# MasterBin-IIAU/Unicorn

Measured on NVIDIA H100. Metric: frames/sec, higher is better.
Workload: dtype bf16

## Files before the change

unicorn_b200/csrc/mlp_fused.cu:

```cuda
#include <algorithm>
#include "uc_ptx.cuh"
#include "uc_common.h"
#include "../../include/unicorn_b200.h"
#include "uc_epilogue.cuh"

namespace uc {

constexpr int kMlpRows = 128;
constexpr int kMlpHC = 64;
constexpr int kMlpConsumers = 2;
constexpr int kMlpThreads = (1 + kMlpConsumers) * 128;

template <int C>
struct MlpCfg {
  static constexpr int KB = (C + 63) / 64;
  static constexpr int A_BYTES = KB * kMlpRows * 128;
  static constexpr int W1_BYTES = KB * kMlpHC * 128;
  static constexpr int NH = C > 256 ? 2 : 1;
  static constexpr int N2 = C / NH;
  static constexpr int W2_BYTES = N2 * 128;
  static constexpr int NCHUNK = 4 * C / kMlpHC;
  static constexpr int STEPS = NH * NCHUNK;
  static constexpr int AS = C <= 192 ? 2 : 1;
  static constexpr int WS = C <= 256 ? 2 : 1;
  static constexpr int SMEM = AS * A_BYTES + WS * (W1_BYTES + W2_BYTES) + 1024 + 512;
  static constexpr int CPT = C / 16;
};

struct alignas(64) MlpParams {
  CUtensorMap tmA, tmW1, tmW2;
  const float* c1;
  const float* b2;
  const float* gamma;
  uint16_t* x;
  int M, m_tiles;
  float ln_eps;
};

enum { A_FULL = 0, A_EMPTY = 2, W1_FULL = 4, W1_EMPTY = 6, W2_FULL = 8, W2_EMPTY = 10, MLP_NBARS = 12 };

template <int C>
__global__ void __launch_bounds__(kMlpThreads, 1) convnext_mlp_kernel(const __grid_constant__ MlpParams p) {
  using Cfg = MlpCfg<C>;
  extern __shared__ uint8_t smem_raw[];
  uint8_t* smem = reinterpret_cast<uint8_t*>((reinterpret_cast<uintptr_t>(smem_raw) + 1023) & ~uintptr_t(1023));
  uint8_t* sA = smem;
  uint8_t* sW1 = sA + Cfg::AS * Cfg::A_BYTES;
  uint8_t* sW2 = sW1 + Cfg::WS * Cfg::W1_BYTES;
  uint64_t* bar = reinterpret_cast<uint64_t*>(sW2 + Cfg::WS * Cfg::W2_BYTES);
  const int wg = threadIdx.x >> 7, warp = threadIdx.x >> 5, lane = threadIdx.x & 31;

  if (threadIdx.x == 0) {
    prefetch_tmap(&p.tmA);
    prefetch_tmap(&p.tmW1);
    prefetch_tmap(&p.tmW2);
    for (int i = 0; i < 2; ++i) {
      mbar_init(&bar[A_FULL + i], 1);
      mbar_init(&bar[A_EMPTY + i], kMlpConsumers);
      mbar_init(&bar[W1_FULL + i], 1);
      mbar_init(&bar[W1_EMPTY + i], kMlpConsumers);
      mbar_init(&bar[W2_FULL + i], 1);
      mbar_init(&bar[W2_EMPTY + i], kMlpConsumers);
    }
    fence_barrier_init();
  }
  __syncthreads();
  pdl_wait();
  pdl_launch_dependents();

  const int n_local = (p.m_tiles - static_cast<int>(blockIdx.x) + static_cast<int>(gridDim.x) - 1) / static_cast<int>(gridDim.x);
  auto tile_of = [&](int i) { return static_cast<int>(blockIdx.x) + i * static_cast<int>(gridDim.x); };

  if (wg == 0) {
    regs_dealloc<40>();
    if (warp != 0) return;
    auto load_a = [&](int i) {
      const int ab = i % Cfg::AS;
      mbar_wait(&bar[A_EMPTY + ab], ((i / Cfg::AS) & 1) ^ 1);
      if (elect_one()) {
        mbar_arrive_expect_tx(&bar[A_FULL + ab], Cfg::A_BYTES);
#pragma unroll
        for (int kb = 0; kb < Cfg::KB; ++kb)
          tma_load_2d(sA + ab * Cfg::A_BYTES + kb * (kMlpRows * 128), &p.tmA, &bar[A_FULL + ab], kb * 64, tile_of(i) * kMlpRows);
      }
      __syncwarp();
    };
    auto load_w = [&](int g) {
      const int s = g % Cfg::WS, ph = (g / Cfg::WS) & 1, j = g % Cfg::NCHUNK, nh = (g / Cfg::NCHUNK) % Cfg::NH;
      mbar_wait(&bar[W1_EMPTY + s], ph ^ 1);
      if (elect_one()) {
        mbar_arrive_expect_tx(&bar[W1_FULL + s], Cfg::W1_BYTES);
#pragma unroll
        for (int kb = 0; kb < Cfg::KB; ++kb)
          tma_load_2d(sW1 + s * Cfg::W1_BYTES + kb * (kMlpHC * 128), &p.tmW1, &bar[W1_FULL + s], kb * 64, j * kMlpHC);
      }
      __syncwarp();
      mbar_wait(&bar[W2_EMPTY + s], ph ^ 1);
      if (elect_one()) {
        mbar_arrive_expect_tx(&bar[W2_FULL + s], Cfg::W2_BYTES);
        tma_load_2d(sW2 + s * Cfg::W2_BYTES, &p.tmW2, &bar[W2_FULL + s], j * kMlpHC, nh * Cfg::N2);
      }
      __syncwarp();
    };
    const int total = n_local * Cfg::STEPS;
    if (n_local > 0) load_a(0);
    for (int g = 0; g < total; ++g) {
      load_w(g);
      const int i = g / Cfg::STEPS, r = g % Cfg::STEPS;
      if (r == (Cfg::AS == 2 ? 0 : Cfg::STEPS - 1) && i + 1 < n_local) load_a(i + 1);
    }
    return;
  }
  regs_alloc<232>();
  const int c = wg - 1, ct = threadIdx.x & 127;
  const int g8 = lane >> 2, t = lane & 3;
  const int rl = (warp & 3) * 16 + g8;
  const int lr = c * 64 + (ct >> 1), lp = ct & 1;
  auto layer_norm_tile = [&](int ab) {
    uint8_t* a = sA + ab * Cfg::A_BYTES + lr * 128;
    auto chunk_ptr = [&](int cc) {
      const int gc = lp * Cfg::CPT + cc;
      return reinterpret_cast<uint4*>(a + (gc >> 3) * (kMlpRows * 128) + (((gc & 7) ^ (lr & 7)) << 4));
    };
    float s1 = 0.f;
#pragma unroll 4
    for (int cc = 0; cc < Cfg::CPT; ++cc) {
      const uint4 v = *chunk_ptr(cc);
      s1 += (bf16lo(v.x) + bf16hi(v.x)) + (bf16lo(v.y) + bf16hi(v.y)) + (bf16lo(v.z) + bf16hi(v.z)) + (bf16lo(v.w) + bf16hi(v.w));
    }
    s1 += __shfl_xor_sync(0xffffffffu, s1, 1);
    const float mean = s1 * (1.f / C);
    float s2 = 0.f;
#pragma unroll 4
    for (int cc = 0; cc < Cfg::CPT; ++cc) {
      const uint4 v = *chunk_ptr(cc);
      const uint32_t w[4] = {v.x, v.y, v.z, v.w};
#pragma unroll
      for (int e = 0; e < 4; ++e) {
        const float d0 = bf16lo(w[e]) - mean, d1 = bf16hi(w[e]) - mean;
        s2 = fmaf(d0, d0, s2);
        s2 = fmaf(d1, d1, s2);
      }
    }
    s2 += __shfl_xor_sync(0xffffffffu, s2, 1);
    const float rstd = rsqrtf(s2 * (1.f / C) + p.ln_eps);
#pragma unroll 4
    for (int cc = 0; cc < Cfg::CPT; ++cc) {
      uint4* ptr = chunk_ptr(cc);
      const uint4 v = *ptr;
      const uint32_t w[4] = {v.x, v.y, v.z, v.w};
      uint32_t o[4];
#pragma unroll
      for (int e = 0; e < 4; ++e) o[e] = pack2_fast((bf16lo(w[e]) - mean) * rstd, (bf16hi(w[e]) - mean) * rstd, false);
      *ptr = make_uint4(o[0], o[1], o[2], o[3]);
    }
    fence_proxy_async();
    named_sync(1 + c, 128);
  };
  const uint64_t a_desc0 = wgmma_desc_sw128(smem_u32(sA + c * 64 * 128)), w1_desc0 = wgmma_desc_sw128(smem_u32(sW1));
  const uint64_t w2_desc0 = wgmma_desc_sw128(smem_u32(sW2));
  float acc2[Cfg::N2 / 2];
  int g = 0;
  for (int i = 0; i < n_local; ++i) {
    const int ab = i % Cfg::AS;
    mbar_wait(&bar[A_FULL + ab], (i / Cfg::AS) & 1);
    layer_norm_tile(ab);
#pragma unroll 1
   for (int nh = 0; nh < Cfg::NH; ++nh) {
    for (int j = 0; j < Cfg::NCHUNK; ++j, ++g) {
      const int ws = g % Cfg::WS, wph = (g / Cfg::WS) & 1;
      float acc1[kMlpHC / 2];
      mbar_wait(&bar[W1_FULL + ws], wph);
      wgmma_fence();
#pragma unroll
      for (int kb = 0; kb < Cfg::KB; ++kb) {
        const uint64_t ad = a_desc0 + static_cast<uint64_t>((ab * Cfg::A_BYTES + kb * (kMlpRows * 128)) >> 4);
        const uint64_t bd = w1_desc0 + static_cast<uint64_t>((ws * Cfg::W1_BYTES + kb * (kMlpHC * 128)) >> 4);
#pragma unroll
        for (int k = 0; k < 4; ++k) wgmma_ss<kMlpHC, false>(acc1, ad + 2 * k, bd + 2 * k, (kb | k) != 0 ? 1u : 0u);
      }
      wgmma_commit();
      wgmma_wait<0>();
      wgmma_fence_regs(acc1);
      if (ct == 0) {
        mbar_arrive(&bar[W1_EMPTY + ws]);
        if (nh == Cfg::NH - 1 && j == Cfg::NCHUNK - 1) mbar_arrive(&bar[A_EMPTY + ab]);
      }
      uint32_t hf[4][4];
#pragma unroll
      for (int kk = 0; kk < 4; ++kk) {
#pragma unroll
        for (int half = 0; half < 2; ++half) {
          const int i8 = 2 * kk + half;
          const float2 bb = __ldg(reinterpret_cast<const float2*>(p.c1 + j * kMlpHC + 8 * i8 + 2 * t));
          const f32x2 h0 = gelu2(add2(pk2(acc1[4 * i8], acc1[4 * i8 + 1]), pk2(bb.x, bb.y)));
          const f32x2 h1 = gelu2(add2(pk2(acc1[4 * i8 + 2], acc1[4 * i8 + 3]), pk2(bb.x, bb.y)));
          hf[kk][2 * half] = pack2_fast(lo2(h0), hi2(h0), false);
          hf[kk][2 * half + 1] = pack2_fast(lo2(h1), hi2(h1), false);
        }
      }
      mbar_wait(&bar[W2_FULL + ws], wph);
      wgmma_fence();
      const uint64_t bd2 = w2_desc0 + static_cast<uint64_t>((ws * Cfg::W2_BYTES) >> 4);
#pragma unroll
      for (int kk = 0; kk < 4; ++kk) wgmma_rs_bf16<Cfg::N2>(acc2, hf[kk], bd2 + 2 * kk, (j | kk) != 0 ? 1u : 0u);
      wgmma_commit();
      wgmma_wait<0>();
      wgmma_fence_regs(acc2);
      if (ct == 0) mbar_arrive(&bar[W2_EMPTY + ws]);
    }
    const long grow0 = static_cast<long>(tile_of(i)) * kMlpRows + c * 64 + rl;
#pragma unroll
    for (int i8 = 0; i8 < Cfg::N2 / 8; ++i8) {
      const int col = nh * Cfg::N2 + 8 * i8 + 2 * t;
      const float2 b = __ldg(reinterpret_cast<const float2*>(p.b2 + col)), gm = __ldg(reinterpret_cast<const float2*>(p.gamma + col));
#pragma unroll
      for (int h = 0; h < 2; ++h) {
        const long grow = grow0 + 8 * h;
        if (grow < p.M) {
          uint32_t* xp = reinterpret_cast<uint32_t*>(p.x + grow * C + col);
          const uint32_t rw = *xp;
          f32x2 v = add2(pk2(acc2[4 * i8 + 2 * h], acc2[4 * i8 + 2 * h + 1]), pk2(b.x, b.y));
          v = mul2(v, pk2(gm.x, gm.y));
          v = add2(v, pk2(bf16lo(rw), bf16hi(rw)));
          *xp = pack2_fast(lo2(v), hi2(v), false);
        }
      }
    }
   }
  }
}

template <int C>
static int launch_mlp(MlpParams& p, cudaStream_t stream) {
  using Cfg = MlpCfg<C>;
  static PerDeviceFlag attr_dev;
  bool& attr = attr_dev.get();
  auto kern = convnext_mlp_kernel<C>;
  if (!attr) {
    cudaError_t e = cudaFuncSetAttribute(kern, cudaFuncAttributeMaxDynamicSharedMemorySize, Cfg::SMEM);
    if (e != cudaSuccess) return set_error(static_cast<int>(e), "uc_convnext_mlp: cudaFuncSetAttribute: %s", cudaGetErrorString(e));
    attr = true;
  }
  const int grid = std::min(p.m_tiles, num_sms());
  cudaError_t e = launch_pdl(kern, dim3(grid), dim3(kMlpThreads), Cfg::SMEM, stream, p);
  if (e != cudaSuccess) return set_error(static_cast<int>(e), "uc_convnext_mlp<%d> launch: %s", C, cudaGetErrorString(e));
  return check_launch("uc_convnext_mlp");
}

}

using namespace uc;

extern "C" int uc_convnext_mlp_supported(int C) { return C == 96 || C == 192 || C == 256 || C == 384; }

extern "C" int uc_convnext_mlp(const void* t_bf16, const void* w1f_bf16, const float* c1, const void* w2_bf16, const float* b2,
                               const float* gamma, void* x_bf16, int M, int C, float ln_eps, void* stream_v) {
  cudaStream_t stream = static_cast<cudaStream_t>(stream_v);
  if (!t_bf16 || !w1f_bf16 || !c1 || !w2_bf16 || !b2 || !gamma || !x_bf16) return set_error(UC_EINVAL, "uc_convnext_mlp: null pointer");
  if (!uc_convnext_mlp_supported(C)) return set_error(UC_EINVAL, "uc_convnext_mlp: C = %d not supported (96, 192, 256, 384)", C);
  if (M < 1) return set_error(UC_EINVAL, "uc_convnext_mlp: empty map");
  if ((reinterpret_cast<uintptr_t>(t_bf16) | reinterpret_cast<uintptr_t>(w1f_bf16) | reinterpret_cast<uintptr_t>(w2_bf16)) & 15 ||
      (reinterpret_cast<uintptr_t>(x_bf16) | reinterpret_cast<uintptr_t>(c1) | reinterpret_cast<uintptr_t>(b2) | reinterpret_cast<uintptr_t>(gamma)) & 31)
    return set_error(UC_EINVAL, "uc_convnext_mlp: t / weights 16-byte, x / biases 32-byte aligned");
  if (t_bf16 == x_bf16) return set_error(UC_EINVAL, "uc_convnext_mlp: t and x must be different maps");
  int rc = ensure_driver();
  if (rc) return rc;
  MlpParams p;
  memset(&p, 0, sizeof(p));
  const uint64_t es = 2;
  {
    uint64_t dims[2] = {static_cast<uint64_t>(C), static_cast<uint64_t>(M)};
    uint64_t strides[1] = {static_cast<uint64_t>(C) * es};
    uint32_t box[2] = {64, kMlpRows};
    rc = encode_tmap(&p.tmA, CU_TENSOR_MAP_DATA_TYPE_BFLOAT16, 2, t_bf16, dims, strides, box);
    if (rc) return rc;
  }
  {
    uint64_t dims[2] = {static_cast<uint64_t>(C), static_cast<uint64_t>(4 * C)};
    uint64_t strides[1] = {static_cast<uint64_t>(C) * es};
    uint32_t box[2] = {64, kMlpHC};
    rc = encode_tmap(&p.tmW1, CU_TENSOR_MAP_DATA_TYPE_BFLOAT16, 2, w1f_bf16, dims, strides, box);
    if (rc) return rc;
  }
  {
    uint64_t dims[2] = {static_cast<uint64_t>(4 * C), static_cast<uint64_t>(C)};
    uint64_t strides[1] = {static_cast<uint64_t>(4 * C) * es};
    uint32_t box[2] = {kMlpHC, static_cast<uint32_t>(C > 256 ? C / 2 : C)};
    rc = encode_tmap(&p.tmW2, CU_TENSOR_MAP_DATA_TYPE_BFLOAT16, 2, w2_bf16, dims, strides, box);
    if (rc) return rc;
  }
  p.c1 = c1; p.b2 = b2; p.gamma = gamma;
  p.x = static_cast<uint16_t*>(x_bf16);
  p.M = M;
  p.m_tiles = (M + kMlpRows - 1) / kMlpRows;
  p.ln_eps = ln_eps;
  return C == 96 ? launch_mlp<96>(p, stream) : C == 192 ? launch_mlp<192>(p, stream) : C == 256 ? launch_mlp<256>(p, stream) : launch_mlp<384>(p, stream);
}
```

unicorn_b200/csrc/uc_ptx.cuh:

```cuda
#pragma once
#include <cuda_runtime.h>
#include <cuda_bf16.h>
#include <cuda_fp16.h>
#include <cuda.h>
#include <stdint.h>
#include <stdio.h>
#include "uc_wgmma.cuh"

namespace uc {

__device__ __forceinline__ uint32_t smem_u32(const void* p) {
  return static_cast<uint32_t>(__cvta_generic_to_shared(p));
}

__device__ __forceinline__ bool elect_one() {
  uint32_t pred;
  asm volatile(
      "{\n\t.reg .pred p;\n\t"
      "elect.sync _|p, 0xffffffff;\n\t"
      "selp.u32 %0, 1, 0, p;\n\t}"
      : "=r"(pred));
  return pred != 0;
}

__device__ __forceinline__ void mbar_init(uint64_t* bar, uint32_t count) {
  asm volatile("mbarrier.init.shared::cta.b64 [%0], %1;" ::"r"(smem_u32(bar)), "r"(count) : "memory");
}
__device__ __forceinline__ void fence_barrier_init() {
  asm volatile("fence.mbarrier_init.release.cluster;" ::: "memory");
}
__device__ __forceinline__ void fence_proxy_async() {
  asm volatile("fence.proxy.async.shared::cta;" ::: "memory");
}
__device__ __forceinline__ void mbar_arrive_expect_tx(uint64_t* bar, uint32_t bytes) {
  asm volatile("mbarrier.arrive.expect_tx.shared::cta.b64 _, [%0], %1;" ::"r"(smem_u32(bar)), "r"(bytes)
               : "memory");
}
__device__ __forceinline__ void mbar_arrive(uint64_t* bar) {
  asm volatile("mbarrier.arrive.shared::cta.b64 _, [%0];" ::"r"(smem_u32(bar)) : "memory");
}
__device__ __forceinline__ bool mbar_try_wait(uint64_t* bar, uint32_t parity) {
  uint32_t ok;
  asm volatile(
      "{\n\t.reg .pred p;\n\t"
      "mbarrier.try_wait.parity.shared::cta.b64 p, [%1], %2;\n\t"
      "selp.u32 %0, 1, 0, p;\n\t}"
      : "=r"(ok)
      : "r"(smem_u32(bar)), "r"(parity)
      : "memory");
  return ok != 0;
}
__device__ __forceinline__ void mbar_wait(uint64_t* bar, uint32_t parity) {
  if (mbar_try_wait(bar, parity)) return;
  long long t0 = clock64();
  uint32_t spins = 0;
  while (!mbar_try_wait(bar, parity)) {
    if ((++spins & 0x3FF) == 0 && (clock64() - t0) > 4000000000LL) __trap();
  }
}

__device__ __forceinline__ void prefetch_tmap(const CUtensorMap* m) {
  asm volatile("prefetch.tensormap [%0];" ::"l"(reinterpret_cast<uint64_t>(m)) : "memory");
}
__device__ __forceinline__ void tma_load_2d(void* smem, const CUtensorMap* m, uint64_t* bar, int c0, int c1) {
  asm volatile(
      "cp.async.bulk.tensor.2d.shared::cluster.global.mbarrier::complete_tx::bytes [%0], [%1, {%3, %4}], [%2];" ::"r"(
          smem_u32(smem)),
      "l"(reinterpret_cast<uint64_t>(m)), "r"(smem_u32(bar)), "r"(c0), "r"(c1)
      : "memory");
}
__device__ __forceinline__ void tma_load_3d(void* smem, const CUtensorMap* m, uint64_t* bar, int c0, int c1, int c2) {
  asm volatile(
      "cp.async.bulk.tensor.3d.shared::cluster.global.mbarrier::complete_tx::bytes [%0], [%1, {%3, %4, %5}], [%2];" ::
          "r"(smem_u32(smem)),
      "l"(reinterpret_cast<uint64_t>(m)), "r"(smem_u32(bar)), "r"(c0), "r"(c1), "r"(c2)
      : "memory");
}
__device__ __forceinline__ void tma_load_4d(void* smem, const CUtensorMap* m, uint64_t* bar, int c0, int c1, int c2,
                                            int c3) {
  asm volatile(
      "cp.async.bulk.tensor.4d.shared::cluster.global.mbarrier::complete_tx::bytes [%0], [%1, {%3, %4, %5, %6}], "
      "[%2];" ::"r"(smem_u32(smem)),
      "l"(reinterpret_cast<uint64_t>(m)), "r"(smem_u32(bar)), "r"(c0), "r"(c1), "r"(c2), "r"(c3)
      : "memory");
}

__device__ __forceinline__ void tma_load_3d_mc(void* smem, const CUtensorMap* m, uint64_t* bar, int c0, int c1, int c2,
                                               uint16_t cta_mask) {
  asm volatile(
      "cp.async.bulk.tensor.3d.shared::cluster.global.mbarrier::complete_tx::bytes.multicast::cluster [%0], [%1, {%3, %4, "
      "%5}], [%2], %6;" ::"r"(smem_u32(smem)),
      "l"(reinterpret_cast<uint64_t>(m)), "r"(smem_u32(bar)), "r"(c0), "r"(c1), "r"(c2), "h"(cta_mask)
      : "memory");
}
__device__ __forceinline__ uint32_t cluster_ctarank() {
  uint32_t r;
  asm volatile("mov.u32 %0, %%cluster_ctarank;" : "=r"(r));
  return r;
}
__device__ __forceinline__ void cluster_sync_all() {
  asm volatile("barrier.cluster.arrive.release.aligned;\nbarrier.cluster.wait.acquire.aligned;" ::: "memory");
}
__device__ __forceinline__ void mbar_arrive_remote(uint64_t* bar, uint32_t rank) {
  asm volatile(
      "{\n\t.reg .b32 ra;\n\t"
      "mapa.shared::cluster.u32 ra, %0, %1;\n\t"
      "mbarrier.arrive.release.cluster.shared::cluster.b64 _, [ra];\n\t}" ::"r"(smem_u32(bar)),
      "r"(rank)
      : "memory");
}

__device__ __forceinline__ void tma_store_4d(const CUtensorMap* m, const void* smem, int c0, int c1, int c2, int c3) {
  asm volatile("cp.async.bulk.tensor.4d.global.shared::cta.bulk_group [%0, {%2, %3, %4, %5}], [%1];" ::"l"(
                   reinterpret_cast<uint64_t>(m)),
               "r"(smem_u32(smem)), "r"(c0), "r"(c1), "r"(c2), "r"(c3)
               : "memory");
}
__device__ __forceinline__ void tma_store_commit() { asm volatile("cp.async.bulk.commit_group;" ::: "memory"); }
__device__ __forceinline__ void tma_store_wait_read() { asm volatile("cp.async.bulk.wait_group.read 0;" ::: "memory"); }
__device__ __forceinline__ void tma_store_wait_all() { asm volatile("cp.async.bulk.wait_group 0;" ::: "memory"); }

__device__ __forceinline__ void wgmma_fence() { asm volatile("wgmma.fence.sync.aligned;" ::: "memory"); }
__device__ __forceinline__ void wgmma_commit() { asm volatile("wgmma.commit_group.sync.aligned;" ::: "memory"); }
template <int N>
__device__ __forceinline__ void wgmma_wait() { asm volatile("wgmma.wait_group.sync.aligned %0;" ::"n"(N) : "memory"); }
template <int K>
__device__ __forceinline__ void wgmma_fence_regs(float (&d)[K]) {
#pragma unroll
  for (int i = 0; i < K; ++i) asm volatile("" : "+f"(d[i])::"memory");
}
template <int R>
__device__ __forceinline__ void regs_dealloc() { asm volatile("setmaxnreg.dec.sync.aligned.u32 %0;" ::"n"(R)); }
template <int R>
__device__ __forceinline__ void regs_alloc() { asm volatile("setmaxnreg.inc.sync.aligned.u32 %0;" ::"n"(R)); }
__device__ __forceinline__ void named_sync(int id, int count) { asm volatile("bar.sync %0, %1;" ::"r"(id), "r"(count) : "memory"); }
__device__ __forceinline__ void named_arrive(int id, int count) { asm volatile("bar.arrive %0, %1;" ::"r"(id), "r"(count) : "memory"); }

__device__ __forceinline__ uint64_t wgmma_desc_sw128(uint32_t smem_addr) {
  uint64_t d = 0;
  d |= static_cast<uint64_t>((smem_addr & 0x3FFFF) >> 4);
  d |= static_cast<uint64_t>(1) << 16;
  d |= static_cast<uint64_t>(1024 >> 4) << 32;
  d |= static_cast<uint64_t>(1) << 62;
  return d;
}

}
```

Baseline: 179.0.

## Split fused MLP across consumer warpgroups via shared hidden buffer for wide channels

For C=384, and for C=256 when there are few row tiles, the kernel switches to 64-row tiles. The two consumer warpgroups alternate computing hidden chunks, which they stage through a 4-slot swizzled shared-memory buffer. Each warpgroup then runs the second GEMM on its own half of the output columns, replacing the earlier two-pass N-half loop that recomputed the first GEMM. A second producer warp now loads W2 separately. This removes the redundant first-GEMM work and gives more tiles, and so more CTAs, for small M, at the cost of extra shared-memory traffic and more mbarrier synchronisation.

```diff
diff --git a/unicorn_b200/csrc/mlp_fused.cu b/unicorn_b200/csrc/mlp_fused.cu
--- a/unicorn_b200/csrc/mlp_fused.cu
+++ b/unicorn_b200/csrc/mlp_fused.cu
@@ -11,20 +11,26 @@
 constexpr int kMlpConsumers = 2;
 constexpr int kMlpThreads = (1 + kMlpConsumers) * 128;
 
-template <int C>
+inline bool mlp_split(int C, int M, int sms) { return C == 384 || (C == 256 && (M + 63) / 64 <= sms); }
+
+template <int C, bool SPLIT_>
 struct MlpCfg {
+  static constexpr bool SPLIT = SPLIT_;
+  static constexpr int ROWS = SPLIT ? 64 : kMlpRows;
   static constexpr int KB = (C + 63) / 64;
-  static constexpr int A_BYTES = KB * kMlpRows * 128;
+  static constexpr int A_BYTES = KB * ROWS * 128;
   static constexpr int W1_BYTES = KB * kMlpHC * 128;
-  static constexpr int NH = C > 256 ? 2 : 1;
-  static constexpr int N2 = C / NH;
-  static constexpr int W2_BYTES = N2 * 128;
+  static constexpr int N2 = SPLIT ? C / 2 : C;
+  static constexpr int W2_BYTES = C * 128;
   static constexpr int NCHUNK = 4 * C / kMlpHC;
-  static constexpr int STEPS = NH * NCHUNK;
   static constexpr int AS = C <= 192 ? 2 : 1;
-  static constexpr int WS = C <= 256 ? 2 : 1;
-  static constexpr int SMEM = AS * A_BYTES + WS * (W1_BYTES + W2_BYTES) + 1024 + 512;
+  static constexpr int W1S = 2;
+  static constexpr int W2S = C <= 256 ? 2 : 1;
+  static constexpr int HS = SPLIT ? 4 : 0;
+  static constexpr int H_BYTES = ROWS * 128;
+  static constexpr int SMEM = AS * A_BYTES + W1S * W1_BYTES + W2S * W2_BYTES + HS * H_BYTES + 1024 + 512;
   static constexpr int CPT = C / 16;
+  static_assert(NCHUNK % 2 == 0 && SMEM <= 227 * 1024, "MlpCfg");
 };
 
 struct alignas(64) MlpParams {
@@ -37,17 +43,18 @@
   float ln_eps;
 };
 
-enum { A_FULL = 0, A_EMPTY = 2, W1_FULL = 4, W1_EMPTY = 6, W2_FULL = 8, W2_EMPTY = 10, MLP_NBARS = 12 };
-
-template <int C>
+enum { A_FULL = 0, A_EMPTY = 2, W1_FULL = 4, W1_EMPTY = 6, W2_FULL = 8, W2_EMPTY = 10, H_FULL = 12, H_EMPTY = 16, MLP_NBARS = 20 };
+
+template <int C, bool SPLIT>
 __global__ void __launch_bounds__(kMlpThreads, 1) convnext_mlp_kernel(const __grid_constant__ MlpParams p) {
-  using Cfg = MlpCfg<C>;
+  using Cfg = MlpCfg<C, SPLIT>;
   extern __shared__ uint8_t smem_raw[];
   uint8_t* smem = reinterpret_cast<uint8_t*>((reinterpret_cast<uintptr_t>(smem_raw) + 1023) & ~uintptr_t(1023));
   uint8_t* sA = smem;
   uint8_t* sW1 = sA + Cfg::AS * Cfg::A_BYTES;
-  uint8_t* sW2 = sW1 + Cfg::WS * Cfg::W1_BYTES;
-  uint64_t* bar = reinterpret_cast<uint64_t*>(sW2 + Cfg::WS * Cfg::W2_BYTES);
+  uint8_t* sW2 = sW1 + Cfg::W1S * Cfg::W1_BYTES;
+  uint8_t* sH = sW2 + Cfg::W2S * Cfg::W2_BYTES;
+  uint64_t* bar = reinterpret_cast<uint64_t*>(sH + Cfg::HS * Cfg::H_BYTES);
   const int wg = threadIdx.x >> 7, warp = threadIdx.x >> 5, lane = threadIdx.x & 31;
 
   if (threadIdx.x == 0) {
@@ -58,9 +65,13 @@
       mbar_init(&bar[A_FULL + i], 1);
       mbar_init(&bar[A_EMPTY + i], kMlpConsumers);
       mbar_init(&bar[W1_FULL + i], 1);
-      mbar_init(&bar[W1_EMPTY + i], kMlpConsumers);
+      mbar_init(&bar[W1_EMPTY + i], Cfg::SPLIT ? 1 : kMlpConsumers);
       mbar_init(&bar[W2_FULL + i], 1);
       mbar_init(&bar[W2_EMPTY + i], kMlpConsumers);
+    }
+    for (int i = 0; i < 4; ++i) {
+      mbar_init(&bar[H_FULL + i], 128);
+      mbar_init(&bar[H_EMPTY + i], kMlpConsumers);
     }
     fence_barrier_init();
   }
@@ -73,7 +84,7 @@
 
   if (wg == 0) {
     regs_dealloc<40>();
-    if (warp != 0) return;
+    if (warp > (Cfg::SPLIT ? 1 : 0)) return;
     auto load_a = [&](int i) {
       const int ab = i % Cfg::AS;
       mbar_wait(&bar[A_EMPTY + ab], ((i / Cfg::AS) & 1) ^ 1);
@@ -81,12 +92,12 @@
         mbar_arrive_expect_tx(&bar[A_FULL + ab], Cfg::A_BYTES);
 #pragma unroll
         for (int kb = 0; kb < Cfg::KB; ++kb)
-          tma_load_2d(sA + ab * Cfg::A_BYTES + kb * (kMlpRows * 128), &p.tmA, &bar[A_FULL + ab], kb * 64, tile_of(i) * kMlpRows);
+          tma_load_2d(sA + ab * Cfg::A_BYTES + kb * (Cfg::ROWS * 128), &p.tmA, &bar[A_FULL + ab], kb * 64, tile_of(i) * Cfg::ROWS);
       }
       __syncwarp();
     };
-    auto load_w = [&](int g) {
-      const int s = g % Cfg::WS, ph = (g / Cfg::WS) & 1, j = g % Cfg::NCHUNK, nh = (g / Cfg::NCHUNK) % Cfg::NH;
+    auto load_w1 = [&](int g) {
+      const int s = g % Cfg::W1S, ph = (g / Cfg::W1S) & 1, j = g % Cfg::NCHUNK;
       mbar_wait(&bar[W1_EMPTY + s], ph ^ 1);
       if (elect_one()) {
         mbar_arrive_expect_tx(&bar[W1_FULL + s], Cfg::W1_BYTES);
@@ -95,19 +106,29 @@
           tma_load_2d(sW1 + s * Cfg::W1_BYTES + kb * (kMlpHC * 128), &p.tmW1, &bar[W1_FULL + s], kb * 64, j * kMlpHC);
       }
       __syncwarp();
+    };
+    auto load_w2 = [&](int g) {
+      const int s = g % Cfg::W2S, ph = (g / Cfg::W2S) & 1, j = g % Cfg::NCHUNK;
       mbar_wait(&bar[W2_EMPTY + s], ph ^ 1);
       if (elect_one()) {
         mbar_arrive_expect_tx(&bar[W2_FULL + s], Cfg::W2_BYTES);
-        tma_load_2d(sW2 + s * Cfg::W2_BYTES, &p.tmW2, &bar[W2_FULL + s], j * kMlpHC, nh * Cfg::N2);
+#pragma unroll
+        for (int h = 0; h < C / Cfg::N2; ++h)
+          tma_load_2d(sW2 + s * Cfg::W2_BYTES + h * (Cfg::N2 * 128), &p.tmW2, &bar[W2_FULL + s], j * kMlpHC, h * Cfg::N2);
       }
       __syncwarp();
     };
-    const int total = n_local * Cfg::STEPS;
+    const int total = n_local * Cfg::NCHUNK;
+    if (Cfg::SPLIT && warp == 1) {
+      for (int g = 0; g < total; ++g) load_w2(g);
+      return;
+    }
     if (n_local > 0) load_a(0);
     for (int g = 0; g < total; ++g) {
-      load_w(g);
-      const int i = g / Cfg::STEPS, r = g % Cfg::STEPS;
-      if (r == (Cfg::AS == 2 ? 0 : Cfg::STEPS - 1) && i + 1 < n_local) load_a(i + 1);
+      load_w1(g);
+      if (!Cfg::SPLIT) load_w2(g);
+      const int i = g / Cfg::NCHUNK, r = g % Cfg::NCHUNK;
+      if (r == (Cfg::AS == 2 ? 0 : Cfg::NCHUNK - 1) && i + 1 < n_local) load_a(i + 1);
     }
     return;
   }
@@ -115,104 +136,132 @@
   const int c = wg - 1, ct = threadIdx.x & 127;
   const int g8 = lane >> 2, t = lane & 3;
   const int rl = (warp & 3) * 16 + g8;
-  const int lr = c * 64 + (ct >> 1), lp = ct & 1;
+  const int lr = c * (Cfg::ROWS / 2) + (ct >> 1), lp = ct & 1;
   auto layer_norm_tile = [&](int ab) {
     uint8_t* a = sA + ab * Cfg::A_BYTES + lr * 128;
     auto chunk_ptr = [&](int cc) {
       const int gc = lp * Cfg::CPT + cc;
-      return reinterpret_cast<uint4*>(a + (gc >> 3) * (kMlpRows * 128) + (((gc & 7) ^ (lr & 7)) << 4));
+      return reinterpret_cast<uint4*>(a + (gc >> 3) * (Cfg::ROWS * 128) + (((gc & 7) ^ (lr & 7)) << 4));
     };
-    float s1 = 0.f;
+    if (ct < Cfg::ROWS) {
+      float s1 = 0.f;
 #pragma unroll 4
-    for (int cc = 0; cc < Cfg::CPT; ++cc) {
-      const uint4 v = *chunk_ptr(cc);
-      s1 += (bf16lo(v.x) + bf16hi(v.x)) + (bf16lo(v.y) + bf16hi(v.y)) + (bf16lo(v.z) + bf16hi(v.z)) + (bf16lo(v.w) + bf16hi(v.w));
-    }
-    s1 += __shfl_xor_sync(0xffffffffu, s1, 1);
-    const float mean = s1 * (1.f / C);
-    float s2 = 0.f;
+      for (int cc = 0; cc < Cfg::CPT; ++cc) {
+        const uint4 v = *chunk_ptr(cc);
+        s1 += (bf16lo(v.x) + bf16hi(v.x)) + (bf16lo(v.y) + bf16hi(v.y)) + (bf16lo(v.z) + bf16hi(v.z)) + (bf16lo(v.w) + bf16hi(v.w));
+      }
+      s1 += __shfl_xor_sync(0xffffffffu, s1, 1);
+      const float mean = s1 * (1.f / C);
+      float s2 = 0.f;
 #pragma unroll 4
-    for (int cc = 0; cc < Cfg::CPT; ++cc) {
-      const uint4 v = *chunk_ptr(cc);
-      const uint32_t w[4] = {v.x, v.y, v.z, v.w};
-#pragma unroll
-      for (int e = 0; e < 4; ++e) {
-        const float d0 = bf16lo(w[e]) - mean, d1 = bf16hi(w[e]) - mean;
-        s2 = fmaf(d0, d0, s2);
-        s2 = fmaf(d1, d1, s2);
-      }
-    }
-    s2 += __shfl_xor_sync(0xffffffffu, s2, 1);
-    const float rstd = rsqrtf(s2 * (1.f / C) + p.ln_eps);
+      for (int cc = 0; cc < Cfg::CPT; ++cc) {
+        const uint4 v = *chunk_ptr(cc);
+        const uint32_t w[4] = {v.x, v.y, v.z, v.w};
+#pragma unroll
+        for (int e = 0; e < 4; ++e) {
+          const float d0 = bf16lo(w[e]) - mean, d1 = bf16hi(w[e]) - mean;
+          s2 = fmaf(d0, d0, s2);
+          s2 = fmaf(d1, d1, s2);
+        }
+      }
+      s2 += __shfl_xor_sync(0xffffffffu, s2, 1);
+      const float rstd = rsqrtf(s2 * (1.f / C) + p.ln_eps);
 #pragma unroll 4
-    for (int cc = 0; cc < Cfg::CPT; ++cc) {
-      uint4* ptr = chunk_ptr(cc);
-      const uint4 v = *ptr;
-      const uint32_t w[4] = {v.x, v.y, v.z, v.w};
-      uint32_t o[4];
-#pragma unroll
-      for (int e = 0; e < 4; ++e) o[e] = pack2_fast((bf16lo(w[e]) - mean) * rstd, (bf16hi(w[e]) - mean) * rstd, false);
-      *ptr = make_uint4(o[0], o[1], o[2], o[3]);
-    }
-    fence_proxy_async();
-    named_sync(1 + c, 128);
+      for (int cc = 0; cc < Cfg::CPT; ++cc) {
+        uint4* ptr = chunk_ptr(cc);
+        const uint4 v = *ptr;
+        const uint32_t w[4] = {v.x, v.y, v.z, v.w};
+        uint32_t o[4];
+#pragma unroll
+        for (int e = 0; e < 4; ++e) o[e] = pack2_fast((bf16lo(w[e]) - mean) * rstd, (bf16hi(w[e]) - mean) * rstd, false);
+        *ptr = make_uint4(o[0], o[1], o[2], o[3]);
+      }
+      fence_proxy_async();
+    }
+    if constexpr (Cfg::SPLIT) named_sync(3, 256);
+    else named_sync(1 + c, 128);
   };
-  const uint64_t a_desc0 = wgmma_desc_sw128(smem_u32(sA + c * 64 * 128)), w1_desc0 = wgmma_desc_sw128(smem_u32(sW1));
-  const uint64_t w2_desc0 = wgmma_desc_sw128(smem_u32(sW2));
+  const uint64_t a_desc0 = wgmma_desc_sw128(smem_u32(sA + (Cfg::SPLIT ? 0 : c * 64 * 128))), w1_desc0 = wgmma_desc_sw128(smem_u32(sW1));
+  const uint64_t w2_desc0 = wgmma_desc_sw128(smem_u32(sW2 + (Cfg::SPLIT ? c * Cfg::N2 * 128 : 0)));
+  const uint64_t h_desc0 = wgmma_desc_sw128(smem_u32(sH));
   float acc2[Cfg::N2 / 2];
   int g = 0;
   for (int i = 0; i < n_local; ++i) {
     const int ab = i % Cfg::AS;
     mbar_wait(&bar[A_FULL + ab], (i / Cfg::AS) & 1);
     layer_norm_tile(ab);
-#pragma unroll 1
-   for (int nh = 0; nh < Cfg::NH; ++nh) {
     for (int j = 0; j < Cfg::NCHUNK; ++j, ++g) {
-      const int ws = g % Cfg::WS, wph = (g / Cfg::WS) & 1;
-      float acc1[kMlpHC / 2];
-      mbar_wait(&bar[W1_FULL + ws], wph);
-      wgmma_fence();
-#pragma unroll
-      for (int kb = 0; kb < Cfg::KB; ++kb) {
-        const uint64_t ad = a_desc0 + static_cast<uint64_t>((ab * Cfg::A_BYTES + kb * (kMlpRows * 128)) >> 4);
-        const uint64_t bd = w1_desc0 + static_cast<uint64_t>((ws * Cfg::W1_BYTES + kb * (kMlpHC * 128)) >> 4);
-#pragma unroll
-        for (int k = 0; k < 4; ++k) wgmma_ss<kMlpHC, false>(acc1, ad + 2 * k, bd + 2 * k, (kb | k) != 0 ? 1u : 0u);
-      }
-      wgmma_commit();
-      wgmma_wait<0>();
-      wgmma_fence_regs(acc1);
-      if (ct == 0) {
-        mbar_arrive(&bar[W1_EMPTY + ws]);
-        if (nh == Cfg::NH - 1 && j == Cfg::NCHUNK - 1) mbar_arrive(&bar[A_EMPTY + ab]);
-      }
+      const int hs = g % 4, hph = (g / 4) & 1;
       uint32_t hf[4][4];
-#pragma unroll
-      for (int kk = 0; kk < 4; ++kk) {
-#pragma unroll
-        for (int half = 0; half < 2; ++half) {
-          const int i8 = 2 * kk + half;
-          const float2 bb = __ldg(reinterpret_cast<const float2*>(p.c1 + j * kMlpHC + 8 * i8 + 2 * t));
-          const f32x2 h0 = gelu2(add2(pk2(acc1[4 * i8], acc1[4 * i8 + 1]), pk2(bb.x, bb.y)));
-          const f32x2 h1 = gelu2(add2(pk2(acc1[4 * i8 + 2], acc1[4 * i8 + 3]), pk2(bb.x, bb.y)));
-          hf[kk][2 * half] = pack2_fast(lo2(h0), hi2(h0), false);
-          hf[kk][2 * half + 1] = pack2_fast(lo2(h1), hi2(h1), false);
-        }
-      }
-      mbar_wait(&bar[W2_FULL + ws], wph);
-      wgmma_fence();
-      const uint64_t bd2 = w2_desc0 + static_cast<uint64_t>((ws * Cfg::W2_BYTES) >> 4);
-#pragma unroll
-      for (int kk = 0; kk < 4; ++kk) wgmma_rs_bf16<Cfg::N2>(acc2, hf[kk], bd2 + 2 * kk, (j | kk) != 0 ? 1u : 0u);
+      if (!Cfg::SPLIT || (j & 1) == c) {
+        const int ws = g % Cfg::W1S, wph = (g / Cfg::W1S) & 1;
+        float acc1[kMlpHC / 2];
+        mbar_wait(&bar[W1_FULL + ws], wph);
+        wgmma_fence();
+#pragma unroll
+        for (int kb = 0; kb < Cfg::KB; ++kb) {
+          const uint64_t ad = a_desc0 + static_cast<uint64_t>((ab * Cfg::A_BYTES + kb * (Cfg::ROWS * 128)) >> 4);
+          const uint64_t bd = w1_desc0 + static_cast<uint64_t>((ws * Cfg::W1_BYTES + kb * (kMlpHC * 128)) >> 4);
+#pragma unroll
+          for (int k = 0; k < 4; ++k) wgmma_ss<kMlpHC, false>(acc1, ad + 2 * k, bd + 2 * k, (kb | k) != 0 ? 1u : 0u);
+        }
+        wgmma_commit();
+        wgmma_wait<0>();
+        wgmma_fence_regs(acc1);
+        if (ct == 0) {
+          mbar_arrive(&bar[W1_EMPTY + ws]);
+          if (j >= Cfg::NCHUNK - (Cfg::SPLIT ? 2 : 1)) mbar_arrive(&bar[A_EMPTY + ab]);
+        }
+#pragma unroll
+        for (int kk = 0; kk < 4; ++kk) {
+#pragma unroll
+          for (int half = 0; half < 2; ++half) {
+            const int i8 = 2 * kk + half;
+            const float2 bb = __ldg(reinterpret_cast<const float2*>(p.c1 + j * kMlpHC + 8 * i8 + 2 * t));
+            const f32x2 h0 = gelu2(add2(pk2(acc1[4 * i8], acc1[4 * i8 + 1]), pk2(bb.x, bb.y)));
+            const f32x2 h1 = gelu2(add2(pk2(acc1[4 * i8 + 2], acc1[4 * i8 + 3]), pk2(bb.x, bb.y)));
+            hf[kk][2 * half] = pack2_fast(lo2(h0), hi2(h0), false);
+            hf[kk][2 * half + 1] = pack2_fast(lo2(h1), hi2(h1), false);
+          }
+        }
+        if constexpr (Cfg::SPLIT) {
+          mbar_wait(&bar[H_EMPTY + hs], hph ^ 1);
+          uint8_t* hrow = sH + hs * Cfg::H_BYTES + rl * 128 + 4 * t;
+#pragma unroll
+          for (int kk = 0; kk < 4; ++kk)
+#pragma unroll
+            for (int q = 0; q < 4; ++q)
+              *reinterpret_cast<uint32_t*>(hrow + (q & 1) * (8 * 128) + (((2 * kk + (q >> 1)) ^ g8) << 4)) = hf[kk][q];
+          fence_proxy_async();
+          mbar_arrive(&bar[H_FULL + hs]);
+        }
+      }
+      const int ws2 = g % Cfg::W2S;
+      mbar_wait(&bar[W2_FULL + ws2], (g / Cfg::W2S) & 1);
+      const uint64_t bd2 = w2_desc0 + static_cast<uint64_t>((ws2 * Cfg::W2_BYTES) >> 4);
+      if constexpr (Cfg::SPLIT) {
+        mbar_wait(&bar[H_FULL + hs], hph);
+        wgmma_fence();
+        const uint64_t hd = h_desc0 + static_cast<uint64_t>((hs * Cfg::H_BYTES) >> 4);
+#pragma unroll
+        for (int kk = 0; kk < 4; ++kk) wgmma_ss<Cfg::N2, false>(acc2, hd + 2 * kk, bd2 + 2 * kk, (j | kk) != 0 ? 1u : 0u);
+      } else {
+        wgmma_fence();
+#pragma unroll
+        for (int kk = 0; kk < 4; ++kk) wgmma_rs_bf16<Cfg::N2>(acc2, hf[kk], bd2 + 2 * kk, (j | kk) != 0 ? 1u : 0u);
+      }
       wgmma_commit();
       wgmma_wait<0>();
       wgmma_fence_regs(acc2);
-      if (ct == 0) mbar_arrive(&bar[W2_EMPTY + ws]);
-    }
-    const long grow0 = static_cast<long>(tile_of(i)) * kMlpRows + c * 64 + rl;
+      if (ct == 0) {
+        mbar_arrive(&bar[W2_EMPTY + ws2]);
+        if (Cfg::SPLIT) mbar_arrive(&bar[H_EMPTY + hs]);
+      }
+    }
+    const long grow0 = static_cast<long>(tile_of(i)) * Cfg::ROWS + (Cfg::SPLIT ? 0 : c * 64) + rl;
 #pragma unroll
     for (int i8 = 0; i8 < Cfg::N2 / 8; ++i8) {
-      const int col = nh * Cfg::N2 + 8 * i8 + 2 * t;
+      const int col = (Cfg::SPLIT ? c * Cfg::N2 : 0) + 8 * i8 + 2 * t;
       const float2 b = __ldg(reinterpret_cast<const float2*>(p.b2 + col)), gm = __ldg(reinterpret_cast<const float2*>(p.gamma + col));
 #pragma unroll
       for (int h = 0; h < 2; ++h) {
@@ -227,16 +276,15 @@
         }
       }
     }
-   }
   }
 }
 
-template <int C>
+template <int C, bool SPLIT>
 static int launch_mlp(MlpParams& p, cudaStream_t stream) {
-  using Cfg = MlpCfg<C>;
+  using Cfg = MlpCfg<C, SPLIT>;
   static PerDeviceFlag attr_dev;
   bool& attr = attr_dev.get();
-  auto kern = convnext_mlp_kernel<C>;
+  auto kern = convnext_mlp_kernel<C, SPLIT>;
   if (!attr) {
     cudaError_t e = cudaFuncSetAttribute(kern, cudaFuncAttributeMaxDynamicSharedMemorySize, Cfg::SMEM);
     if (e != cudaSuccess) return set_error(static_cast<int>(e), "uc_convnext_mlp: cudaFuncSetAttribute: %s", cudaGetErrorString(e));
@@ -266,13 +314,15 @@
   if (t_bf16 == x_bf16) return set_error(UC_EINVAL, "uc_convnext_mlp: t and x must be different maps");
   int rc = ensure_driver();
   if (rc) return rc;
+  const bool split = mlp_split(C, M, num_sms());
+  const int rows = split ? 64 : kMlpRows;
   MlpParams p;
   memset(&p, 0, sizeof(p));
   const uint64_t es = 2;
   {
     uint64_t dims[2] = {static_cast<uint64_t>(C), static_cast<uint64_t>(M)};
     uint64_t strides[1] = {static_cast<uint64_t>(C) * es};
-    uint32_t box[2] = {64, kMlpRows};
+    uint32_t box[2] = {64, static_cast<uint32_t>(rows)};
     rc = encode_tmap(&p.tmA, CU_TENSOR_MAP_DATA_TYPE_BFLOAT16, 2, t_bf16, dims, strides, box);
     if (rc) return rc;
   }
@@ -286,14 +336,17 @@
   {
     uint64_t dims[2] = {static_cast<uint64_t>(4 * C), static_cast<uint64_t>(C)};
     uint64_t strides[1] = {static_cast<uint64_t>(4 * C) * es};
-    uint32_t box[2] = {kMlpHC, static_cast<uint32_t>(C > 256 ? C / 2 : C)};
+    uint32_t box[2] = {kMlpHC, static_cast<uint32_t>(split ? C / 2 : C)};
     rc = encode_tmap(&p.tmW2, CU_TENSOR_MAP_DATA_TYPE_BFLOAT16, 2, w2_bf16, dims, strides, box);
     if (rc) return rc;
   }
   p.c1 = c1; p.b2 = b2; p.gamma = gamma;
   p.x = static_cast<uint16_t*>(x_bf16);
   p.M = M;
-  p.m_tiles = (M + kMlpRows - 1) / kMlpRows;
+  p.m_tiles = (M + rows - 1) / rows;
   p.ln_eps = ln_eps;
-  return C == 96 ? launch_mlp<96>(p, stream) : C == 192 ? launch_mlp<192>(p, stream) : C == 256 ? launch_mlp<256>(p, stream) : launch_mlp<384>(p, stream);
+  if (C == 96) return launch_mlp<96, false>(p, stream);
+  if (C == 192) return launch_mlp<192, false>(p, stream);
+  if (C == 256) return split ? launch_mlp<256, true>(p, stream) : launch_mlp<256, false>(p, stream);
+  return launch_mlp<384, true>(p, stream);
 }
```

Result: no change. 180.4, median of 6 (+0.8%).

## Pipeline GEMM2 with next GEMM1, TMA residual load/store, ping-pong consumer turns

Applied to the files above, without the earlier changes.

Restructures the fused ConvNeXt MLP kernel so each chunk's second GEMM is issued together with the next chunk's first GEMM, overlapping GELU with tensor-core work. The residual epilogue no longer does scattered global read-modify-writes. A new producer warp TMA-loads the residual tile into shared memory (reusing the A buffer when possible), consumers update it in place, and the warp TMA-stores it back. Named-barrier turn-taking between the two consumer warpgroups alternates their wgmma issue. This adds barriers, shared memory for the staging buffer, and more complex synchronization in exchange for less epilogue memory stall.

```diff
diff --git a/unicorn_b200/csrc/mlp_fused.cu b/unicorn_b200/csrc/mlp_fused.cu
--- a/unicorn_b200/csrc/mlp_fused.cu
+++ b/unicorn_b200/csrc/mlp_fused.cu
@@ -23,12 +23,15 @@
   static constexpr int STEPS = NH * NCHUNK;
   static constexpr int AS = C <= 192 ? 2 : 1;
   static constexpr int WS = C <= 256 ? 2 : 1;
-  static constexpr int SMEM = AS * A_BYTES + WS * (W1_BYTES + W2_BYTES) + 1024 + 512;
+  static constexpr bool X_IN_A = NH == 1;
+  static constexpr int XKB = X_IN_A ? KB : N2 / 64;
+  static constexpr int X_BYTES = X_IN_A ? 0 : XKB * kMlpRows * 128;
+  static constexpr int SMEM = AS * A_BYTES + WS * (W1_BYTES + W2_BYTES) + X_BYTES + 1024 + 512;
   static constexpr int CPT = C / 16;
 };
 
 struct alignas(64) MlpParams {
-  CUtensorMap tmA, tmW1, tmW2;
+  CUtensorMap tmA, tmW1, tmW2, tmX;
   const float* c1;
   const float* b2;
   const float* gamma;
@@ -37,7 +40,9 @@
   float ln_eps;
 };
 
-enum { A_FULL = 0, A_EMPTY = 2, W1_FULL = 4, W1_EMPTY = 6, W2_FULL = 8, W2_EMPTY = 10, MLP_NBARS = 12 };
+enum { A_FULL = 0, A_EMPTY = 2, W1_FULL = 4, W1_EMPTY = 6, W2_FULL = 8, W2_EMPTY = 10, X_FULL = 12, A_READ = 14, MLP_NBARS = 16 };
+constexpr int kMlpXDoneBar = 3;
+constexpr int kMlpTurnBar = 5;
 
 template <int C>
 __global__ void __launch_bounds__(kMlpThreads, 1) convnext_mlp_kernel(const __grid_constant__ MlpParams p) {
@@ -47,16 +52,20 @@
   uint8_t* sA = smem;
   uint8_t* sW1 = sA + Cfg::AS * Cfg::A_BYTES;
   uint8_t* sW2 = sW1 + Cfg::WS * Cfg::W1_BYTES;
-  uint64_t* bar = reinterpret_cast<uint64_t*>(sW2 + Cfg::WS * Cfg::W2_BYTES);
+  uint8_t* sX = sW2 + Cfg::WS * Cfg::W2_BYTES;
+  uint64_t* bar = reinterpret_cast<uint64_t*>(sX + Cfg::X_BYTES);
   const int wg = threadIdx.x >> 7, warp = threadIdx.x >> 5, lane = threadIdx.x & 31;
 
   if (threadIdx.x == 0) {
     prefetch_tmap(&p.tmA);
     prefetch_tmap(&p.tmW1);
     prefetch_tmap(&p.tmW2);
+    prefetch_tmap(&p.tmX);
     for (int i = 0; i < 2; ++i) {
       mbar_init(&bar[A_FULL + i], 1);
-      mbar_init(&bar[A_EMPTY + i], kMlpConsumers);
+      mbar_init(&bar[A_EMPTY + i], Cfg::X_IN_A ? 1 : kMlpConsumers);
+      mbar_init(&bar[X_FULL + i], 1);
+      mbar_init(&bar[A_READ + i], 1);
       mbar_init(&bar[W1_FULL + i], 1);
       mbar_init(&bar[W1_EMPTY + i], kMlpConsumers);
       mbar_init(&bar[W2_FULL + i], 1);
@@ -73,18 +82,68 @@
 
   if (wg == 0) {
     regs_dealloc<40>();
+    if (warp == 1) {
+      auto load_a = [&](int i) {
+        const int ab = i % Cfg::AS;
+        mbar_wait(&bar[A_EMPTY + ab], ((i / Cfg::AS) & 1) ^ 1);
+        if (lane == 0) {
+          mbar_arrive_expect_tx(&bar[A_FULL + ab], Cfg::A_BYTES);
+#pragma unroll
+          for (int kb = 0; kb < Cfg::KB; ++kb)
+            tma_load_2d(sA + ab * Cfg::A_BYTES + kb * (kMlpRows * 128), &p.tmA, &bar[A_FULL + ab], kb * 64, tile_of(i) * kMlpRows);
+        }
+        __syncwarp();
+      };
+      auto stage_of = [&](int i) { return Cfg::X_IN_A ? sA + (i % Cfg::AS) * Cfg::A_BYTES : sX; };
+      auto load_x = [&](int i, int nh, int c) {
+        if (lane == 0) {
+          mbar_arrive_expect_tx(&bar[X_FULL + c], Cfg::XKB * 64 * 128);
+#pragma unroll
+          for (int kb = 0; kb < Cfg::XKB; ++kb)
+            tma_load_2d(stage_of(i) + kb * (kMlpRows * 128) + c * 64 * 128, &p.tmX, &bar[X_FULL + c], nh * Cfg::N2 + kb * 64,
+                        tile_of(i) * kMlpRows + c * 64);
+        }
+        __syncwarp();
+      };
+      auto store_x = [&](int i, int nh, int c) {
+        named_sync(kMlpXDoneBar + c, 128 + 32);
+        if (lane == 0) {
+#pragma unroll
+          for (int kb = 0; kb < Cfg::XKB; ++kb)
+            tma_store_2d(&p.tmX, stage_of(i) + kb * (kMlpRows * 128) + c * 64 * 128, nh * Cfg::N2 + kb * 64, tile_of(i) * kMlpRows + c * 64);
+          tma_store_commit();
+        }
+      };
+      if (n_local > 0) load_a(0);
+      for (int i = 0; i < n_local; ++i) {
+        if (Cfg::AS == 2 && i + 1 < n_local) load_a(i + 1);
+        for (int nh = 0; nh < Cfg::NH; ++nh) {
+          if (Cfg::X_IN_A) {
+            for (int c = 0; c < kMlpConsumers; ++c) {
+              mbar_wait(&bar[A_READ + c], i & 1);
+              load_x(i, nh, c);
+            }
+          } else {
+            if (lane == 0) tma_store_wait_read();
+            __syncwarp();
+            for (int c = 0; c < kMlpConsumers; ++c) load_x(i, nh, c);
+            if (nh == Cfg::NH - 1 && i + 1 < n_local) load_a(i + 1);
+          }
+          for (int c = 0; c < kMlpConsumers; ++c) store_x(i, nh, c);
+        }
+        if (Cfg::X_IN_A) {
+          if (lane == 0) {
+            tma_store_wait_read();
+            mbar_arrive(&bar[A_EMPTY + i % Cfg::AS]);
+          }
+          __syncwarp();
+          if (Cfg::AS == 1 && i + 1 < n_local) load_a(i + 1);
+        }
+      }
+      if (lane == 0) tma_store_wait_all();
+      return;
+    }
     if (warp != 0) return;
-    auto load_a = [&](int i) {
-      const int ab = i % Cfg::AS;
-      mbar_wait(&bar[A_EMPTY + ab], ((i / Cfg::AS) & 1) ^ 1);
-      if (elect_one()) {
-        mbar_arrive_expect_tx(&bar[A_FULL + ab], Cfg::A_BYTES);
-#pragma unroll
-        for (int kb = 0; kb < Cfg::KB; ++kb)
-          tma_load_2d(sA + ab * Cfg::A_BYTES + kb * (kMlpRows * 128), &p.tmA, &bar[A_FULL + ab], kb * 64, tile_of(i) * kMlpRows);
-      }
-      __syncwarp();
-    };
     auto load_w = [&](int g) {
       const int s = g % Cfg::WS, ph = (g / Cfg::WS) & 1, j = g % Cfg::NCHUNK, nh = (g / Cfg::NCHUNK) % Cfg::NH;
       mbar_wait(&bar[W1_EMPTY + s], ph ^ 1);
@@ -103,12 +162,7 @@
       __syncwarp();
     };
     const int total = n_local * Cfg::STEPS;
-    if (n_local > 0) load_a(0);
-    for (int g = 0; g < total; ++g) {
-      load_w(g);
-      const int i = g / Cfg::STEPS, r = g % Cfg::STEPS;
-      if (r == (Cfg::AS == 2 ? 0 : Cfg::STEPS - 1) && i + 1 < n_local) load_a(i + 1);
-    }
+    for (int g = 0; g < total; ++g) load_w(g);
     return;
   }
   regs_alloc<232>();
@@ -159,74 +213,116 @@
   };
   const uint64_t a_desc0 = wgmma_desc_sw128(smem_u32(sA + c * 64 * 128)), w1_desc0 = wgmma_desc_sw128(smem_u32(sW1));
   const uint64_t w2_desc0 = wgmma_desc_sw128(smem_u32(sW2));
+  auto gemm1 = [&](float (&acc1)[kMlpHC / 2], int ab, int ws) {
+#pragma unroll
+    for (int kb = 0; kb < Cfg::KB; ++kb) {
+      const uint64_t ad = a_desc0 + static_cast<uint64_t>((ab * Cfg::A_BYTES + kb * (kMlpRows * 128)) >> 4);
+      const uint64_t bd = w1_desc0 + static_cast<uint64_t>((ws * Cfg::W1_BYTES + kb * (kMlpHC * 128)) >> 4);
+#pragma unroll
+      for (int k = 0; k < 4; ++k) wgmma_ss<kMlpHC, false>(acc1, ad + 2 * k, bd + 2 * k, (kb | k) != 0 ? 1u : 0u);
+    }
+  };
+  auto gelu_chunk = [&](const float (&acc1)[kMlpHC / 2], int j, uint32_t (&hf)[4][4]) {
+#pragma unroll
+    for (int kk = 0; kk < 4; ++kk) {
+#pragma unroll
+      for (int half = 0; half < 2; ++half) {
+        const int i8 = 2 * kk + half;
+        const float2 bb = __ldg(reinterpret_cast<const float2*>(p.c1 + j * kMlpHC + 8 * i8 + 2 * t));
+        const f32x2 h0 = gelu2(add2(pk2(acc1[4 * i8], acc1[4 * i8 + 1]), pk2(bb.x, bb.y)));
+        const f32x2 h1 = gelu2(add2(pk2(acc1[4 * i8 + 2], acc1[4 * i8 + 3]), pk2(bb.x, bb.y)));
+        hf[kk][2 * half] = pack2_fast(lo2(h0), hi2(h0), false);
+        hf[kk][2 * half + 1] = pack2_fast(lo2(h1), hi2(h1), false);
+      }
+    }
+  };
+  const int srow = (c * 64 + rl) * 128;
   float acc2[Cfg::N2 / 2];
+  float acc1[kMlpHC / 2];
+  uint32_t hf[4][4];
+  constexpr bool kTurns = C != 256;
+  auto take_turn = [&]() {
+    if (kTurns) asm volatile("{\n\t.reg .u32 b;\n\tmov.u32 b, %%tid.x;\n\tshr.u32 b, b, 7;\n\tadd.u32 b, b, %0;\n\tbar.sync b, 256;\n\t}" ::"n"(kMlpTurnBar - 1));
+  };
+  auto pass_turn = [&](bool pass = true) {
+    if (kTurns) asm volatile("{\n\t.reg .u32 b;\n\t.reg .pred p;\n\tmov.u32 b, %%tid.x;\n\tshr.u32 b, b, 7;\n\txor.b32 b, b, 3;\n\tadd.u32 b, b, %0;\n\t"
+                 "setp.ne.s32 p, %1, 0;\n\t@p bar.arrive b, 256;\n\t}" ::"n"(kMlpTurnBar - 1), "r"(static_cast<int>(pass)));
+  };
+  if (kTurns) asm volatile("{\n\t.reg .pred p;\n\tsetp.eq.s32 p, %1, 1;\n\t@p bar.arrive %0, 256;\n\t}" ::"r"(kMlpTurnBar), "r"(c));
   int g = 0;
-  for (int i = 0; i < n_local; ++i) {
+  for (int i = 0; tile_of(i) < p.m_tiles; ++i) {
     const int ab = i % Cfg::AS;
     mbar_wait(&bar[A_FULL + ab], (i / Cfg::AS) & 1);
     layer_norm_tile(ab);
 #pragma unroll 1
    for (int nh = 0; nh < Cfg::NH; ++nh) {
-    for (int j = 0; j < Cfg::NCHUNK; ++j, ++g) {
+    {
       const int ws = g % Cfg::WS, wph = (g / Cfg::WS) & 1;
-      float acc1[kMlpHC / 2];
       mbar_wait(&bar[W1_FULL + ws], wph);
+      take_turn();
       wgmma_fence();
-#pragma unroll
-      for (int kb = 0; kb < Cfg::KB; ++kb) {
-        const uint64_t ad = a_desc0 + static_cast<uint64_t>((ab * Cfg::A_BYTES + kb * (kMlpRows * 128)) >> 4);
-        const uint64_t bd = w1_desc0 + static_cast<uint64_t>((ws * Cfg::W1_BYTES + kb * (kMlpHC * 128)) >> 4);
-#pragma unroll
-        for (int k = 0; k < 4; ++k) wgmma_ss<kMlpHC, false>(acc1, ad + 2 * k, bd + 2 * k, (kb | k) != 0 ? 1u : 0u);
-      }
+      gemm1(acc1, ab, ws);
       wgmma_commit();
       wgmma_wait<0>();
+      pass_turn();
       wgmma_fence_regs(acc1);
-      if (ct == 0) {
-        mbar_arrive(&bar[W1_EMPTY + ws]);
-        if (nh == Cfg::NH - 1 && j == Cfg::NCHUNK - 1) mbar_arrive(&bar[A_EMPTY + ab]);
-      }
-      uint32_t hf[4][4];
-#pragma unroll
-      for (int kk = 0; kk < 4; ++kk) {
-#pragma unroll
-        for (int half = 0; half < 2; ++half) {
-          const int i8 = 2 * kk + half;
-          const float2 bb = __ldg(reinterpret_cast<const float2*>(p.c1 + j * kMlpHC + 8 * i8 + 2 * t));
-          const f32x2 h0 = gelu2(add2(pk2(acc1[4 * i8], acc1[4 * i8 + 1]), pk2(bb.x, bb.y)));
-          const f32x2 h1 = gelu2(add2(pk2(acc1[4 * i8 + 2], acc1[4 * i8 + 3]), pk2(bb.x, bb.y)));
-          hf[kk][2 * half] = pack2_fast(lo2(h0), hi2(h0), false);
-          hf[kk][2 * half + 1] = pack2_fast(lo2(h1), hi2(h1), false);
-        }
-      }
+      if (ct == 0) mbar_arrive(&bar[W1_EMPTY + ws]);
+      gelu_chunk(acc1, 0, hf);
+    }
+    auto gemm2_gemm1 = [&](int j, bool next) {
+      const int ws = g % Cfg::WS, wph = (g / Cfg::WS) & 1;
+      const int ws1 = (g + 1) % Cfg::WS, wph1 = ((g + 1) / Cfg::WS) & 1;
       mbar_wait(&bar[W2_FULL + ws], wph);
+      if (next) mbar_wait(&bar[W1_FULL + ws1], wph1);
+      take_turn();
       wgmma_fence();
       const uint64_t bd2 = w2_desc0 + static_cast<uint64_t>((ws * Cfg::W2_BYTES) >> 4);
 #pragma unroll
       for (int kk = 0; kk < 4; ++kk) wgmma_rs_bf16<Cfg::N2>(acc2, hf[kk], bd2 + 2 * kk, (j | kk) != 0 ? 1u : 0u);
+      if (next) gemm1(acc1, ab, ws1);
       wgmma_commit();
       wgmma_wait<0>();
+      pass_turn(next || c == 0 || nh != Cfg::NH - 1 || tile_of(i + 1) < p.m_tiles);
       wgmma_fence_regs(acc2);
-      if (ct == 0) mbar_arrive(&bar[W2_EMPTY + ws]);
-    }
-    const long grow0 = static_cast<long>(tile_of(i)) * kMlpRows + c * 64 + rl;
-#pragma unroll
-    for (int i8 = 0; i8 < Cfg::N2 / 8; ++i8) {
-      const int col = nh * Cfg::N2 + 8 * i8 + 2 * t;
-      const float2 b = __ldg(reinterpret_cast<const float2*>(p.b2 + col)), gm = __ldg(reinterpret_cast<const float2*>(p.gamma + col));
-#pragma unroll
-      for (int h = 0; h < 2; ++h) {
-        const long grow = grow0 + 8 * h;
-        if (grow < p.M) {
-          uint32_t* xp = reinterpret_cast<uint32_t*>(p.x + grow * C + col);
-          const uint32_t rw = *xp;
-          f32x2 v = add2(pk2(acc2[4 * i8 + 2 * h], acc2[4 * i8 + 2 * h + 1]), pk2(b.x, b.y));
-          v = mul2(v, pk2(gm.x, gm.y));
-          v = add2(v, pk2(bf16lo(rw), bf16hi(rw)));
-          *xp = pack2_fast(lo2(v), hi2(v), false);
-        }
-      }
-    }
+      if (next) wgmma_fence_regs(acc1);
+      if (ct == 0) {
+        mbar_arrive(&bar[W2_EMPTY + ws]);
+        if (next) mbar_arrive(&bar[W1_EMPTY + ws1]);
+        if (next && nh == Cfg::NH - 1 && j + 2 == Cfg::NCHUNK) mbar_arrive(Cfg::X_IN_A ? &bar[A_READ + c] : &bar[A_EMPTY + ab]);
+      }
+      ++g;
+      if (next) gelu_chunk(acc1, j + 1, hf);
+    };
+#pragma unroll 1
+    for (int j = 0; j + 1 < Cfg::NCHUNK; ++j) gemm2_gemm1(j, true);
+    gemm2_gemm1(Cfg::NCHUNK - 1, false);
+    mbar_wait(&bar[X_FULL + c], (i * Cfg::NH + nh) & 1);
+    uint8_t* const stg = (Cfg::X_IN_A ? sA + ab * Cfg::A_BYTES : sX) + srow + 4 * t;
+#pragma unroll
+    for (int kb = 0; kb < Cfg::N2 / 64 + (Cfg::N2 % 64 != 0); ++kb) {
+      constexpr int kI8 = 8;
+      uint32_t rw[kI8][2];
+#pragma unroll
+      for (int q = 0; q < kI8; ++q)
+#pragma unroll
+        for (int h = 0; h < 2; ++h)
+          if (8 * kb + q < Cfg::N2 / 8) rw[q][h] = *reinterpret_cast<const uint32_t*>(stg + kb * (kMlpRows * 128) + h * 8 * 128 + ((q ^ g8) << 4));
+#pragma unroll
+      for (int q = 0; q < kI8; ++q) {
+        const int i8 = 8 * kb + q;
+        if (i8 >= Cfg::N2 / 8) break;
+        const int col = nh * Cfg::N2 + 8 * i8 + 2 * t;
+        const float2 b = __ldg(reinterpret_cast<const float2*>(p.b2 + col)), gm = __ldg(reinterpret_cast<const float2*>(p.gamma + col));
+#pragma unroll
+        for (int h = 0; h < 2; ++h) {
+          const float v0 = acc2[4 * i8 + 2 * h] + b.x, v1 = acc2[4 * i8 + 2 * h + 1] + b.y;
+          *reinterpret_cast<uint32_t*>(stg + kb * (kMlpRows * 128) + h * 8 * 128 + ((q ^ g8) << 4)) =
+              pack2_fast(fmaf(v0, gm.x, bf16lo(rw[q][h])), fmaf(v1, gm.y, bf16hi(rw[q][h])), false);
+        }
+      }
+    }
+    fence_proxy_async();
+    named_arrive(kMlpXDoneBar + c, 128 + 32);
    }
   }
 }
@@ -290,6 +386,13 @@
     rc = encode_tmap(&p.tmW2, CU_TENSOR_MAP_DATA_TYPE_BFLOAT16, 2, w2_bf16, dims, strides, box);
     if (rc) return rc;
   }
+  {
+    uint64_t dims[2] = {static_cast<uint64_t>(C), static_cast<uint64_t>(M)};
+    uint64_t strides[1] = {static_cast<uint64_t>(C) * es};
+    uint32_t box[2] = {64, 64};
+    rc = encode_tmap(&p.tmX, CU_TENSOR_MAP_DATA_TYPE_BFLOAT16, 2, x_bf16, dims, strides, box);
+    if (rc) return rc;
+  }
   p.c1 = c1; p.b2 = b2; p.gamma = gamma;
   p.x = static_cast<uint16_t*>(x_bf16);
   p.M = M;
diff --git a/unicorn_b200/csrc/uc_ptx.cuh b/unicorn_b200/csrc/uc_ptx.cuh
--- a/unicorn_b200/csrc/uc_ptx.cuh
+++ b/unicorn_b200/csrc/uc_ptx.cuh
@@ -116,6 +116,11 @@
                "r"(smem_u32(smem)), "r"(c0), "r"(c1), "r"(c2), "r"(c3)
                : "memory");
 }
+__device__ __forceinline__ void tma_store_2d(const CUtensorMap* m, const void* smem, int c0, int c1) {
+  asm volatile("cp.async.bulk.tensor.2d.global.shared::cta.bulk_group [%0, {%2, %3}], [%1];" ::"l"(reinterpret_cast<uint64_t>(m)),
+               "r"(smem_u32(smem)), "r"(c0), "r"(c1)
+               : "memory");
+}
 __device__ __forceinline__ void tma_store_commit() { asm volatile("cp.async.bulk.commit_group;" ::: "memory"); }
 __device__ __forceinline__ void tma_store_wait_read() { asm volatile("cp.async.bulk.wait_group.read 0;" ::: "memory"); }
 __device__ __forceinline__ void tma_store_wait_all() { asm volatile("cp.async.bulk.wait_group 0;" ::: "memory"); }
```

After: 177.5 before, 181.3 after (median of 6 runs). 2.1% higher.
